# intellerce/controlanimate

Measured on AMD Instinct MI355X. Metric: frames_per_sec, higher is better.
Workload: dtype fp16

## Files before the change

### controlanimate_amd/context.py

```python
from __future__ import annotations

from dataclasses import dataclass, field
from typing import Optional

import torch


@dataclass
class ExecCtx:
    b: int
    f: int
    dtype: torch.dtype
    temb: torch.Tensor
    emb_groups: int
    ehs: Optional[torch.Tensor] = None
    frames_per_kv: int = 1
    kv_mod: int = 0
    gn_frames_per_stat: int = 1
    cache: dict = field(default_factory=dict)

    @property
    def images(self) -> int:
        return self.b * self.f

    def rows_per_emb_group(self, h: int, w: int) -> int:
        return self.images // self.emb_groups * h * w


class Dispatch:
    gemm_ar = True
    ff_fused = True
    tattn_fused = True
    xattn_fused = True
    attn_out_fused = True
    xattn_ip_fused = True
    conv_winograd = True
    gn_winograd = True
    ln_row_sums = True
    repeat_kernel = True
    ln_fold = True
    cfg_shared = True
    cn_cfg_dedup = True
    controlnet_streams = 2


dispatch = Dispatch()
```

### controlanimate_amd/csrc/ca_conv_wino.h

```cpp

template <int DT>
__global__ __launch_bounds__(256) void k_pack_w_wino(const u16* __restrict__ w, u16* __restrict__ dst, int cout, int cin) {
  const int64_t idx = (int64_t)blockIdx.x * 256 + threadIdx.x;
  if (idx >= (int64_t)cout * cin) return;
  const int ci = (int)(idx % cin);
  const int co = (int)(idx / cin);
  float g[3][3];
#pragma unroll
  for (int kh = 0; kh < 3; ++kh)
#pragma unroll
    for (int kw = 0; kw < 3; ++kw) g[kh][kw] = Elem<DT>::to_f(w[((int64_t)co * 9 + kh * 3 + kw) * cin + ci]);
  float t[4][3];
#pragma unroll
  for (int kw = 0; kw < 3; ++kw) {
    t[0][kw] = g[0][kw];
    t[1][kw] = 0.5f * ((g[0][kw] + g[1][kw]) + g[2][kw]);
    t[2][kw] = 0.5f * ((g[0][kw] - g[1][kw]) + g[2][kw]);
    t[3][kw] = g[2][kw];
  }
#pragma unroll
  for (int xi = 0; xi < 4; ++xi) {
    const float u[4] = {t[xi][0], 0.5f * ((t[xi][0] + t[xi][1]) + t[xi][2]), 0.5f * ((t[xi][0] - t[xi][1]) + t[xi][2]), t[xi][2]};
#pragma unroll
    for (int nu = 0; nu < 4; ++nu) dst[((int64_t)(xi * 4 + nu) * cout + co) * cin + ci] = Elem<DT>::from_f(u[nu]);
  }
}

struct WinoParams {
  const u16* x;
  const u16* x2;
  u16* v;
  const u16* mm;
  u16* y;
  const float* bias;
  const float* rowbias;
  const u16* res;
  int64_t ld_res, ld_rowbias;
  int images, h, w, c1, c2, cout;
  int ups;
  int rows_per_group;
  float alpha, post;
  int act;
};

__device__ __forceinline__ unsigned wino_pk_add(unsigned a, unsigned b) {
  unsigned r;
  asm("v_pk_add_f16 %0, %1, %2" : "=v"(r) : "v"(a), "v"(b));
  return r;
}
__device__ __forceinline__ unsigned wino_pk_sub(unsigned a, unsigned b) {
  unsigned r;
  asm("v_pk_add_f16 %0, %1, %2 neg_lo:[0,1] neg_hi:[0,1]" : "=v"(r) : "v"(a), "v"(b));
  return r;
}

template <int DT>
__device__ __forceinline__ unsigned wino_add2(unsigned a, unsigned b) {
  if (DT == CA_F16) return wino_pk_add(a, b);
  return pack2<DT>(Elem<DT>::to_f((u16)(a & 0xffffu)) + Elem<DT>::to_f((u16)(b & 0xffffu)), Elem<DT>::to_f((u16)(a >> 16)) + Elem<DT>::to_f((u16)(b >> 16)));
}
template <int DT>
__device__ __forceinline__ unsigned wino_sub2(unsigned a, unsigned b) {
  if (DT == CA_F16) return wino_pk_sub(a, b);
  return pack2<DT>(Elem<DT>::to_f((u16)(a & 0xffffu)) - Elem<DT>::to_f((u16)(b & 0xffffu)), Elem<DT>::to_f((u16)(a >> 16)) - Elem<DT>::to_f((u16)(b >> 16)));
}

template <int DT>
__global__ __launch_bounds__(256) void k_wino_in(WinoParams p) {
  const int c = p.c1 + p.c2;
  const int chunks = c >> 3;
  const int th = p.h >> 1, tw = p.w >> 1;
  const int64_t tiles = (int64_t)p.images * th * tw;
  const int64_t idx = (int64_t)blockIdx.x * 256 + threadIdx.x;
  if (idx >= tiles * chunks) return;
  const int ck = (int)(idx % chunks);
  const int64_t t = idx / chunks;
  const int tx = (int)(t % tw);
  const int ty = (int)((t / tw) % th);
  const int img = (int)(t / ((int64_t)tw * th));
  const bool second = ck * 8 >= p.c1;
  const u16* src = second ? p.x2 : p.x;
  const int cs = second ? p.c2 : p.c1;
  const int c0 = second ? ck * 8 - p.c1 : ck * 8;
  u32x4 d[4][4];
#pragma unroll
  for (int i = 0; i < 4; ++i) {
    const int hy = 2 * ty - 1 + i;
#pragma unroll
    for (int j = 0; j < 4; ++j) {
      const int wx = 2 * tx - 1 + j;
      const int sh = p.h >> p.ups, sw = p.w >> p.ups;
      d[i][j] = (hy >= 0 && hy < p.h && wx >= 0 && wx < p.w) ? ld16(src + (((int64_t)img * sh + (hy >> p.ups)) * sw + (wx >> p.ups)) * cs + c0) : (u32x4){0u, 0u, 0u, 0u};
    }
  }
  u32x4 r[4][4];
#pragma unroll
  for (int j = 0; j < 4; ++j)
#pragma unroll
    for (int e = 0; e < 4; ++e) {
      r[0][j][e] = wino_sub2<DT>(d[0][j][e], d[2][j][e]);
      r[1][j][e] = wino_add2<DT>(d[1][j][e], d[2][j][e]);
      r[2][j][e] = wino_sub2<DT>(d[2][j][e], d[1][j][e]);
      r[3][j][e] = wino_sub2<DT>(d[1][j][e], d[3][j][e]);
    }
  const int64_t fstride = tiles * c;
  u16* dst = p.v + t * c + ck * 8;
#pragma unroll
  for (int xi = 0; xi < 4; ++xi) {
    u32x4 o[4];
#pragma unroll
    for (int e = 0; e < 4; ++e) {
      o[0][e] = wino_sub2<DT>(r[xi][0][e], r[xi][2][e]);
      o[1][e] = wino_add2<DT>(r[xi][1][e], r[xi][2][e]);
      o[2][e] = wino_sub2<DT>(r[xi][2][e], r[xi][1][e]);
      o[3][e] = wino_sub2<DT>(r[xi][1][e], r[xi][3][e]);
    }
#pragma unroll
    for (int nu = 0; nu < 4; ++nu) st16(dst + (int64_t)(xi * 4 + nu) * fstride, o[nu]);
  }
}

template <int DT>
__global__ __launch_bounds__(256) void k_wino_out(WinoParams p) {
  const int chunks = p.cout >> 3;
  const int th = p.h >> 1, tw = p.w >> 1;
  const int64_t tiles = (int64_t)p.images * th * tw;
  const int64_t idx = (int64_t)blockIdx.x * 256 + threadIdx.x;
  if (idx >= tiles * chunks) return;
  const int ck = (int)(idx % chunks);
  const int64_t t = idx / chunks;
  const int tx = (int)(t % tw);
  const int ty = (int)((t / tw) % th);
  const int img = (int)(t / ((int64_t)tw * th));
  const int64_t fstride = tiles * p.cout;
  const u16* src = p.mm + t * p.cout + ck * 8;
  float s[2][4][8];
#pragma unroll
  for (int nu = 0; nu < 4; ++nu) {
    float m[4][8];
#pragma unroll
    for (int xi = 0; xi < 4; ++xi) unpack8<DT>(ld16(src + (int64_t)(xi * 4 + nu) * fstride), m[xi]);
#pragma unroll
    for (int e = 0; e < 8; ++e) {
      s[0][nu][e] = (m[0][e] + m[1][e]) + m[2][e];
      s[1][nu][e] = (m[1][e] - m[2][e]) - m[3][e];
    }
  }
  const int n0 = ck * 8;
  float bi[8];
#pragma unroll
  for (int e = 0; e < 8; ++e) bi[e] = p.bias ? p.bias[n0 + e] : 0.f;
#pragma unroll
  for (int i = 0; i < 2; ++i)
#pragma unroll
    for (int j = 0; j < 2; ++j) {
      const int64_t m = ((int64_t)img * p.h + 2 * ty + i) * p.w + 2 * tx + j;
      float v[8];
#pragma unroll
      for (int e = 0; e < 8; ++e) v[e] = j == 0 ? (s[i][0][e] + s[i][1][e]) + s[i][2][e] : (s[i][1][e] - s[i][2][e]) - s[i][3][e];
#pragma unroll
      for (int e = 0; e < 8; ++e) v[e] += bi[e];
      if (p.rowbias) {
        const float* rb = p.rowbias + (m / p.rows_per_group) * p.ld_rowbias + n0;
#pragma unroll
        for (int e = 0; e < 8; ++e) v[e] += rb[e];
      }
#pragma unroll
      for (int e = 0; e < 8; ++e) v[e] *= p.alpha;
      if (p.res) {
        float rr[8];
        unpack8<DT>(ld16(p.res + m * p.ld_res + n0), rr);
#pragma unroll
// ... 12 lines not shown
```

### controlanimate_amd/csrc/ca_norm.hip

```cpp
#include "ca_common.h"
#include <stdlib.h>

namespace {

constexpr int GN_MAX_SLOTS = 5;
constexpr int GN_MAX_C = 64 * 8 * GN_MAX_SLOTS;

inline int gn_chunks_rows(int64_t rows_per_stat, int rows_per_chunk) {
  int64_t n = (rows_per_stat + rows_per_chunk - 1) / rows_per_chunk;
  if (n < 16) n = (rows_per_stat + 3) / 4 < 16 ? (rows_per_stat + 3) / 4 : 16;
  if (n < 1) n = 1;
  if (n > 256) n = 256;
  return (int)n;
}
inline int gn_chunks_host(int64_t rows_per_stat) { return gn_chunks_rows(rows_per_stat, 256); }

struct GnParams {
  const u16* x;
  const u16* x2;
  u16* y;
  const float* gamma;
  const float* beta;
  float* partials;
  int c1, c2, groups;
  int64_t rows_per_stat;
  int nchunks;
  int64_t rows_per_chunk;
  float eps;
  int act;
  u16* wino_v;
  int wino_h, wino_w;
};

__host__ __device__ inline int gn_txlog(int c8) {
  int best = 6, best_waste = 1 << 30, best_slots = 0;
  for (int l = 3; l <= 6; ++l) {
    const int tx = 1 << l, slots = (c8 + tx - 1) / tx;
    if (slots > 5) continue;
    const int waste = slots * tx - c8;
    if (waste < best_waste || (waste == best_waste && best_slots != 2 && slots == 2)) {
      best_waste = waste;
      best = l;
      best_slots = slots;
    }
  }
  return best;
}

template <int DT, int txlog, int SLOTS = GN_MAX_SLOTS>
__global__ __launch_bounds__(256) void k_gn_stats(GnParams p) {
  __shared__ float ch_s[GN_MAX_C];
  __shared__ float ch_ss[GN_MAX_C];
  const int C = p.c1 + p.c2, C8 = C >> 3;
// ... 89 lines not shown
      float* out = p.partials + (((int64_t)sg * p.nchunks + chunk) * p.groups + g) * 2;
      out[0] = a;
      out[1] = b;
    }
    return;
  }
#pragma unroll
  for (int k = 0; k < SLOTS; ++k) {
    if ((k << txlog) < C8) {
#pragma unroll
      for (int j = 0; j < 8; ++j) {
#pragma unroll
        for (int off = TX; off < 64; off <<= 1) {
          s[k][j] += __shfl_xor(s[k][j], off);
          ss[k][j] += __shfl_xor(ss[k][j], off);
        }
      }
    }
  }
  for (int w = 0; w < 4; ++w) {
    if (wave == w && lane < TX) {
#pragma unroll
      for (int k = 0; k < SLOTS; ++k) {
        const int c8 = tx + (k << txlog);
        if (c8 < C8) {
#pragma unroll
          for (int j = 0; j < 8; ++j) {
            const int ch = (c8 << 3) + j;
            if (w == 0) {
              ch_s[ch] = s[k][j];
              ch_ss[ch] = ss[k][j];
            } else {
              ch_s[ch] += s[k][j];
              ch_ss[ch] += ss[k][j];
            }
          }
        }
      }
    }
    __syncthreads();
  }
  if (threadIdx.x < p.groups) {
    float a = 0.f, b = 0.f;
    for (int j = 0; j < cpg; ++j) {
      a += ch_s[threadIdx.x * cpg + j];
      b += ch_ss[threadIdx.x * cpg + j];
    }
    float* out = p.partials + (((int64_t)sg * p.nchunks + chunk) * p.groups + threadIdx.x) * 2;
    out[0] = a;
    out[1] = b;
  }
}

template <int DT, int txlog, int SLOTS = GN_MAX_SLOTS>
__global__ __launch_bounds__(256) void k_gn_apply(GnParams p) {
  __shared__ double red[8][64][2];
  __shared__ float gm[64], gr[64];
  const int C = p.c1 + p.c2, C8 = C >> 3;
  constexpr int TX = 1 << txlog, TY = 256 >> txlog;
  const int tx = threadIdx.x & (TX - 1), ty = threadIdx.x >> txlog;
  const int chunk = blockIdx.x, sg = blockIdx.y;
  const int cpg = C / p.groups;
  {
    const int S = p.groups <= 32 ? 8 : 4;
    const int g = threadIdx.x % (256 / S), slot = threadIdx.x / (256 / S);
    if (g < p.groups) {
      double a = 0.0, b = 0.0;
      const float* part = p.partials + ((int64_t)sg * p.nchunks * p.groups + g) * 2;
      for (int k = slot; k < p.nchunks; k += S) {
        const float2 v = *reinterpret_cast<const float2*>(part + (int64_t)k * p.groups * 2);
        a += (double)v.x;
        b += (double)v.y;
      }
      red[slot][g][0] = a;
      red[slot][g][1] = b;
    }
    __syncthreads();
    if (threadIdx.x < p.groups) {
      double a = 0.0, b = 0.0;
      for (int q = 0; q < S; ++q) {
        a += red[q][threadIdx.x][0];
        b += red[q][threadIdx.x][1];
      }
      const double cnt = (double)p.rows_per_stat * (double)cpg;
      const double mean = a / cnt;
      double var = b / cnt - mean * mean;
      if (var < 0.0) var = 0.0;
      gm[threadIdx.x] = (float)mean;
      gr[threadIdx.x] = (float)(1.0 / sqrt(var + (double)p.eps));
    }
    __syncthreads();
  }
  float rs[SLOTS][8], rh[SLOTS][8];
#pragma unroll
  for (int k = 0; k < SLOTS; ++k) {
    const int c8 = tx + (k << txlog);
    if (c8 < C8) {
      const f32x4 g0 = *reinterpret_cast<const f32x4*>(p.gamma + (c8 << 3)), g1 = *reinterpret_cast<const f32x4*>(p.gamma + (c8 << 3) + 4);
      const f32x4 b0 = *reinterpret_cast<const f32x4*>(p.beta + (c8 << 3)), b1 = *reinterpret_cast<const f32x4*>(p.beta + (c8 << 3) + 4);
#pragma unroll
      for (int j = 0; j < 8; ++j) {
        const int gi = ((c8 << 3) + j) / cpg;
        const float scale = gr[gi] * (j < 4 ? g0[j & 3] : g1[j & 3]);
        rs[k][j] = scale;
        rh[k][j] = (j < 4 ? b0[j & 3] : b1[j & 3]) - gm[gi] * scale;
      }
    }
  }
  const int64_t r0 = (int64_t)chunk * p.rows_per_chunk;
  int64_t r1 = r0 + p.rows_per_chunk;
  if (r1 > p.rows_per_stat) r1 = p.rows_per_stat;
  const int64_t base_row = (int64_t)sg * p.rows_per_stat;
  for (int64_t piece = chunk;; piece += 2 * (int64_t)gridDim.x) {
    const int64_t ra = piece * TY + ty, rb = (piece + gridDim.x) * TY + ty;
    if (piece * TY >= p.rows_per_stat) break;
    const bool ok[2] = {ra < p.rows_per_stat, rb < p.rows_per_stat};
    const int64_t rows2[2] = {base_row + ra, base_row + rb};
    u32x4 raw[2][SLOTS];
#pragma unroll
    for (int h = 0; h < 2; ++h)
#pragma unroll
      for (int k = 0; k < SLOTS; ++k) {
        const int c8 = tx + (k << txlog);
        if (c8 < C8 && ok[h]) {
          const int ch = c8 << 3;
          const int64_t rr = rows2[h];
          raw[h][k] = ld16(ch < p.c1 ? p.x + rr * p.c1 + ch : p.x2 + rr * p.c2 + (ch - p.c1));
        }
      }
#pragma unroll
    for (int h = 0; h < 2; ++h)
#pragma unroll
      for (int k = 0; k < SLOTS; ++k) {
        const int c8 = tx + (k << txlog);
        if (c8 < C8 && ok[h]) {
          float f[8];
          unpack8<DT>(raw[h][k], f);
#pragma unroll
          for (int j = 0; j < 8; ++j) {
            const float v = f[j] * rs[k][j] + rh[k][j];
            f[j] = p.act == CA_ACT_SILU ? silu_f(v) : v;
          }
          st16(p.y + rows2[h] * C + (c8 << 3), pack8<DT>(f));
        }
      }
  }
}

constexpr int GNS_MAX = 12;
template <int DT, int NCH = GNS_MAX>
__global__ __launch_bounds__(256) void k_gn_small(GnParams p) {
  __shared__ double red[4][2];
  __shared__ float mr[2];
  const int C = p.c1 + p.c2;
  const int cpg = C / p.groups, q = cpg >> 3;
  const int g = blockIdx.x, sg = blockIdx.y;
  const int total = (int)p.rows_per_stat * q;
  const int64_t base_row = (int64_t)sg * p.rows_per_stat;
  const int lane = threadIdx.x & 63, wave = threadIdx.x >> 6;
  u32x4 raw[NCH];
  float s = 0.f, ss = 0.f;
#pragma unroll
  for (int k = 0; k < NCH; ++k) {
    const int id = threadIdx.x + k * 256;
    if (id < total) {
      const int row = id / q, ch = g * cpg + (id - row * q) * 8;
      const int64_t rr = base_row + row;
      raw[k] = ld16(ch < p.c1 ? p.x + rr * p.c1 + ch : p.x2 + rr * p.c2 + (ch - p.c1));
    }
  }
#pragma unroll
  for (int k = 0; k < NCH; ++k) {
    if (threadIdx.x + k * 256 < total) {
      float f[8];
      unpack8<DT>(raw[k], f);
#pragma unroll
      for (int j = 0; j < 8; ++j) {
        s += f[j];
        ss += f[j] * f[j];
      }
    }
  }
#pragma unroll
  for (int off = 1; off < 64; off <<= 1) {
    s += __shfl_xor(s, off);
    ss += __shfl_xor(ss, off);
  }
  if (lane == 0) {
    red[wave][0] = (double)s;
    red[wave][1] = (double)ss;
  }
  __syncthreads();
  if (threadIdx.x == 0) {
    const double a = red[0][0] + red[1][0] + red[2][0] + red[3][0], b = red[0][1] + red[1][1] + red[2][1] + red[3][1];
    const double cnt = (double)p.rows_per_stat * (double)cpg;
    const double mean = a / cnt;
    double var = b / cnt - mean * mean;
    if (var < 0.0) var = 0.0;
    mr[0] = (float)mean;
    mr[1] = (float)(1.0 / sqrt(var + (double)p.eps));
  }
  __syncthreads();
  const float mean = mr[0], rstd = mr[1];
#pragma unroll
  for (int k = 0; k < NCH; ++k) {
    const int id = threadIdx.x + k * 256;
    if (id < total) {
      const int row = id / q, ch = g * cpg + (id - row * q) * 8;
      const f32x4 g0 = *reinterpret_cast<const f32x4*>(p.gamma + ch), g1 = *reinterpret_cast<const f32x4*>(p.gamma + ch + 4);
      const f32x4 b0 = *reinterpret_cast<const f32x4*>(p.beta + ch), b1 = *reinterpret_cast<const f32x4*>(p.beta + ch + 4);
      float f[8];
      unpack8<DT>(raw[k], f);
#pragma unroll
      for (int j = 0; j < 8; ++j) {
        const float scale = rstd * (j < 4 ? g0[j & 3] : g1[j & 3]);
        const float v = f[j] * scale + ((j < 4 ? b0[j & 3] : b1[j & 3]) - mean * scale);
        f[j] = p.act == CA_ACT_SILU ? silu_f(v) : v;
      }
      st16(p.y + (base_row + row) * C + ch, pack8<DT>(f));
    }
  }
}

__device__ __forceinline__ unsigned gnw_pk_add(unsigned a, unsigned b) {
  unsigned r;
  asm("v_pk_add_f16 %0, %1, %2" : "=v"(r) : "v"(a), "v"(b));
  return r;
}
__device__ __forceinline__ unsigned gnw_pk_sub(unsigned a, unsigned b) {
  unsigned r;
  asm("v_pk_add_f16 %0, %1, %2 neg_lo:[0,1] neg_hi:[0,1]" : "=v"(r) : "v"(a), "v"(b));
  return r;
}
constexpr int GNW_MAX_ROWS = 256, GNW_MAX_CPG = 80;
template <int NCH, int CPG_MAX>
__global__ __launch_bounds__(256) void k_gn_small_wino(GnParams p) {
  constexpr int DT = CA_F16;
  __shared__ double red[4][2];
  __shared__ float mr[2];
  __shared__ __attribute__((aligned(16))) u16 slab[GNW_MAX_ROWS * CPG_MAX];
  const int C = p.c1 + p.c2;
  const int cpg = C / p.groups, q = cpg >> 3;
  const int g = blockIdx.x, sg = blockIdx.y;
  const int total = (int)p.rows_per_stat * q;
  const int64_t base_row = (int64_t)sg * p.rows_per_stat;
  const int lane = threadIdx.x & 63, wave = threadIdx.x >> 6;
  u32x4 raw[NCH];
  float s = 0.f, ss = 0.f;
#pragma unroll
  for (int k = 0; k < NCH; ++k) {
    const int id = threadIdx.x + k * 256;
    if (id < total) {
      const int row = id / q, ch = g * cpg + (id - row * q) * 8;
      const int64_t rr = base_row + row;
      raw[k] = ld16(ch < p.c1 ? p.x + rr * p.c1 + ch : p.x2 + rr * p.c2 + (ch - p.c1));
    }
  }
#pragma unroll
  for (int k = 0; k < NCH; ++k) {
    if (threadIdx.x + k * 256 < total) {
      float f[8];
      unpack8<DT>(raw[k], f);
#pragma unroll
      for (int j = 0; j < 8; ++j) {
        s += f[j];
        ss += f[j] * f[j];
      }
    }
  }
#pragma unroll
  for (int off = 1; off < 64; off <<= 1) {
    s += __shfl_xor(s, off);
    ss += __shfl_xor(ss, off);
  }
  if (lane == 0) {
    red[wave][0] = (double)s;
    red[wave][1] = (double)ss;
  }
  __syncthreads();
  if (threadIdx.x == 0) {
    const double a = red[0][0] + red[1][0] + red[2][0] + red[3][0], b = red[0][1] + red[1][1] + red[2][1] + red[3][1];
    const double cnt = (double)p.rows_per_stat * (double)cpg;
    const double mean = a / cnt;
    double var = b / cnt - mean * mean;
    if (var < 0.0) var = 0.0;
    mr[0] = (float)mean;
    mr[1] = (float)(1.0 / sqrt(var + (double)p.eps));
  }
  __syncthreads();
  const float mean = mr[0], rstd = mr[1];
#pragma unroll
  for (int k = 0; k < NCH; ++k) {
    const int id = threadIdx.x + k * 256;
    if (id < total) {
      const int row = id / q, cq = id - row * q, ch = g * cpg + cq * 8;
      const f32x4 g0 = *reinterpret_cast<const f32x4*>(p.gamma + ch), g1 = *reinterpret_cast<const f32x4*>(p.gamma + ch + 4);
      const f32x4 b0 = *reinterpret_cast<const f32x4*>(p.beta + ch), b1 = *reinterpret_cast<const f32x4*>(p.beta + ch + 4);
      float f[8];
      unpack8<DT>(raw[k], f);
#pragma unroll
      for (int j = 0; j < 8; ++j) {
        const float scale = rstd * (j < 4 ? g0[j & 3] : g1[j & 3]);
        const float v = f[j] * scale + ((j < 4 ? b0[j & 3] : b1[j & 3]) - mean * scale);
        f[j] = p.act == CA_ACT_SILU ? silu_f(v) : v;
      }
      st16(slab + (row * q + cq) * 8, pack8<DT>(f));
    }
  }
  __syncthreads();
  const int th = p.wino_h >> 1, tw = p.wino_w >> 1;
  const int items = th * tw * q;
  const int64_t tiles_total = (int64_t)gridDim.y * th * tw;
  const int64_t fstride = tiles_total * C;
  for (int it = threadIdx.x; it < items; it += 256) {
    const int cq = it % q, t = it / q;
    const int tx = t % tw, ty = t / tw;
    u32x4 d[4][4];
#pragma unroll
    for (int i = 0; i < 4; ++i) {
      const int hy = 2 * ty - 1 + i;
#pragma unroll
      for (int j = 0; j < 4; ++j) {
        const int wx = 2 * tx - 1 + j;
        d[i][j] = (hy >= 0 && hy < p.wino_h && wx >= 0 && wx < p.wino_w) ? ld16(slab + ((hy * p.wino_w + wx) * q + cq) * 8) : (u32x4){0u, 0u, 0u, 0u};
      }
    }
    u32x4 r[4][4];
#pragma unroll
    for (int j = 0; j < 4; ++j)
#pragma unroll
      for (int e = 0; e < 4; ++e) {
        r[0][j][e] = gnw_pk_sub(d[0][j][e], d[2][j][e]);
        r[1][j][e] = gnw_pk_add(d[1][j][e], d[2][j][e]);
        r[2][j][e] = gnw_pk_sub(d[2][j][e], d[1][j][e]);
        r[3][j][e] = gnw_pk_sub(d[1][j][e], d[3][j][e]);
      }
    u16* dst = p.wino_v + ((int64_t)sg * th * tw + t) * C + g * cpg + cq * 8;
#pragma unroll
    for (int xi = 0; xi < 4; ++xi) {
      u32x4 o[4];
#pragma unroll
      for (int e = 0; e < 4; ++e) {
        o[0][e] = gnw_pk_sub(r[xi][0][e], r[xi][2][e]);
        o[1][e] = gnw_pk_add(r[xi][1][e], r[xi][2][e]);
        o[2][e] = gnw_pk_sub(r[xi][2][e], r[xi][1][e]);
        o[3][e] = gnw_pk_sub(r[xi][1][e], r[xi][3][e]);
      }
#pragma unroll
      for (int nu = 0; nu < 4; ++nu) st16(dst + (int64_t)(xi * 4 + nu) * fstride, o[nu]);
    }
  }
}

constexpr int GNU_MAX = 20;
template <int DT, int NCH>
__global__ __launch_bounds__(1024, NCH <= 5 ? 2 : 1) void k_gn_unit(GnParams p, int uc, int units) {
  __shared__ float red[16][4][2];
  __shared__ float mr[4][2];
  __shared__ __attribute__((aligned(16))) float sc[128], sh[128];
  const int C = p.c1 + p.c2;
  const int cpg = C / p.groups, q = uc >> 3, ug = uc / cpg;
  const unsigned bid = blockIdx.x;
  const int nstat = gridDim.x / units;
  int unit, sg;
  if (nstat % 8 == 0) {
    unit = (bid >> 3) % units;
    sg = (bid & 7) + 8 * (bid / (8 * units));
  } else {
    unit = bid % units;
    sg = bid / units;
  }
  const int total = (int)p.rows_per_stat * q;
  const int64_t base_row = (int64_t)sg * p.rows_per_stat;
  const int lane = threadIdx.x & 63, wave = threadIdx.x >> 6;
  u32x4 raw[NCH];
#pragma unroll
  for (int k = 0; k < NCH; ++k) {
    const int id = threadIdx.x + k * 1024;
    if (id < total) {
      const int row = id / q, ch = unit * uc + (id - row * q) * 8;
      const int64_t rr = base_row + row;
      raw[k] = ld16(ch < p.c1 ? p.x + rr * p.c1 + ch : p.x2 + rr * p.c2 + (ch - p.c1));
    }
  }
  float acc[4][2] = {{0.f, 0.f}, {0.f, 0.f}, {0.f, 0.f}, {0.f, 0.f}};
#pragma unroll
  for (int k = 0; k < NCH; ++k) {
    const int id = threadIdx.x + k * 1024;
    if (id < total) {
      const int cq = id % q;
      const int ga = (cq * 8) / cpg, n0 = (ga + 1) * cpg - cq * 8;
      float f[8];
      unpack8<DT>(raw[k], f);
      float lo = 0.f, lo2 = 0.f, hi = 0.f, hi2 = 0.f;
#pragma unroll
      for (int j = 0; j < 8; ++j) {
        if (j < n0) {
          lo += f[j];
          lo2 = fmaf(f[j], f[j], lo2);
        } else {
          hi += f[j];
          hi2 = fmaf(f[j], f[j], hi2);
        }
// ... 310 lines not shown

template <int DT, int L>
void launch_gn_l(bool apply, int slots, const GnParams& p, dim3 grid, hipStream_t st) {
  if (slots <= 2) {
    if (apply) hipLaunchKernelGGL((k_gn_apply<DT, L, 2>), grid, dim3(256), 0, st, p);
    else hipLaunchKernelGGL((k_gn_stats<DT, L, 2>), grid, dim3(256), 0, st, p);
  } else if (slots <= 4) {
    if (apply) hipLaunchKernelGGL((k_gn_apply<DT, L, 4>), grid, dim3(256), 0, st, p);
    else hipLaunchKernelGGL((k_gn_stats<DT, L, 4>), grid, dim3(256), 0, st, p);
  } else {
    if (apply) hipLaunchKernelGGL((k_gn_apply<DT, L, 5>), grid, dim3(256), 0, st, p);
    else hipLaunchKernelGGL((k_gn_stats<DT, L, 5>), grid, dim3(256), 0, st, p);
  }
}

template <int DT>
void launch_gn(bool apply, const GnParams& p, dim3 grid, hipStream_t st) {
  const int c8 = (p.c1 + p.c2) >> 3;
  const int txlog = gn_txlog(c8);
  const int slots = (c8 + (1 << txlog) - 1) >> txlog;
  switch (txlog) {
    case 3: launch_gn_l<DT, 3>(apply, slots, p, grid, st); break;
    case 4: launch_gn_l<DT, 4>(apply, slots, p, grid, st); break;
    case 5: launch_gn_l<DT, 5>(apply, slots, p, grid, st); break;
    default: launch_gn_l<DT, 6>(apply, slots, p, grid, st);
  }
}

extern "C" int ca_groupnorm_stats(const ca_groupnorm_args* a, void* stream) {
  GnParams p{};
  int rc = gn_fill(a, p, "ca_groupnorm_stats");
  if (rc) return rc;
  dim3 grid(p.nchunks, a->images / a->frames_per_stat);
  if (a->dtype == CA_BF16) launch_gn<CA_BF16>(false, p, grid, (hipStream_t)stream);
  else launch_gn<CA_F16>(false, p, grid, (hipStream_t)stream);
  CA_CHECK_LAUNCH("ca_groupnorm_stats");
  return CA_OK;
}

extern "C" int ca_groupnorm_apply(const ca_groupnorm_args* a, void* stream) {
  GnParams p{};
  int rc = gn_fill(a, p, "ca_groupnorm_apply");
  if (rc) return rc;
  CA_REQUIRE(a->y && a->gamma && a->beta, "ca_groupnorm_apply: null operand");
  const int achunks = gn_chunks_rows(p.rows_per_stat, p.rows_per_stat >= 2048 ? 128 : 64);
  p.rows_per_chunk = (p.rows_per_stat + achunks - 1) / achunks;
  dim3 grid(achunks, a->images / a->frames_per_stat);
  if (a->dtype == CA_BF16) launch_gn<CA_BF16>(true, p, grid, (hipStream_t)stream);
  else launch_gn<CA_F16>(true, p, grid, (hipStream_t)stream);
  CA_CHECK_LAUNCH("ca_groupnorm_apply");
  return CA_OK;
}

extern "C" int ca_groupnorm_wino_supported(const ca_groupnorm_args* a) {
  if (!a || !a->x || !a->gamma || !a->beta || !a->wino_v || a->dtype != CA_F16 || a->frames_per_stat != 1) return 0;
  if (a->images <= 0 || a->c1 <= 0 || a->c1 % 8 || a->c2 < 0 || a->c2 % 8 || (a->c2 && !a->x2) || a->groups <= 0) return 0;
  const int C = a->c1 + a->c2;
  if (C % a->groups) return 0;
  const int cpg = C / a->groups;
  if (cpg % 8 || cpg > GNW_MAX_CPG || (a->c2 != 0 && a->c1 % cpg != 0)) return 0;
  if (a->wino_h < 2 || a->wino_w < 2 || (a->wino_h & 1) || (a->wino_w & 1) || a->wino_h * a->wino_w != a->hw || a->hw > GNW_MAX_ROWS) return 0;
  if ((int64_t)a->hw * (cpg >> 3) > 256 * GNS_MAX) return 0;
  if ((((uintptr_t)a->wino_v | (uintptr_t)a->x | (uintptr_t)a->x2) & 15) != 0) return 0;
  return 1;
}

extern "C" int ca_groupnorm(const ca_groupnorm_args* a, void* stream) {
  GnParams p{};
  if (a && a->wino_v) {
    CA_REQUIRE(ca_groupnorm_wino_supported(a), "ca_groupnorm: wino_v with arguments outside the fused form (fp16, per-image statistics, even image of <= 256 pixels, "
                                                "<= 80 channels per group in whole 8-channel chunks): ask ca_groupnorm_wino_supported() first");
    p.x = (const u16*)a->x;
    p.x2 = (const u16*)a->x2;
    p.gamma = a->gamma;
    p.beta = a->beta;
    p.c1 = a->c1, p.c2 = a->c2, p.groups = a->groups;
    p.rows_per_stat = a->hw;
    p.eps = a->eps;
    p.act = a->act;
    p.wino_v = (u16*)a->wino_v;
    p.wino_h = a->wino_h, p.wino_w = a->wino_w;
    {
      const int cpg_w = (a->c1 + a->c2) / a->groups;
      const int64_t per_thread = ((int64_t)a->hw * (cpg_w >> 3) + 255) / 256;
      const dim3 grid_w(a->groups, a->images);
      hipStream_t st_w = (hipStream_t)stream;
#define CA_GNW_CASE(N)                                                                                  \
  if (cpg_w <= 40) hipLaunchKernelGGL((k_gn_small_wino<N, 40>), grid_w, dim3(256), 0, st_w, p);         \
  else hipLaunchKernelGGL((k_gn_small_wino<N, GNW_MAX_CPG>), grid_w, dim3(256), 0, st_w, p);
      if (per_thread <= 2) { CA_GNW_CASE(2) }
      else if (per_thread <= 5) { CA_GNW_CASE(5) }
      else { CA_GNW_CASE(GNS_MAX) }
#undef CA_GNW_CASE
    }
    CA_CHECK_LAUNCH("ca_groupnorm(wino)");
    return CA_OK;
  }
  int rc = gn_fill(a, p, "ca_groupnorm");
  if (rc) return rc;
  CA_REQUIRE(a->y && a->gamma && a->beta, "ca_groupnorm: null operand");
  if (gn_small_ok(p)) {
    const dim3 grid(p.groups, a->images / a->frames_per_stat);
    const int64_t per_thread = (p.rows_per_stat * ((p.c1 + p.c2) / p.groups >> 3) + 255) / 256;
#define CA_GNS_CASE(N)                                                                                                     \
  if (a->dtype == CA_BF16) hipLaunchKernelGGL((k_gn_small<CA_BF16, N>), grid, dim3(256), 0, (hipStream_t)stream, p);       \
  else hipLaunchKernelGGL((k_gn_small<CA_F16, N>), grid, dim3(256), 0, (hipStream_t)stream, p);
    if (per_thread <= 2) { CA_GNS_CASE(2) }
    else if (per_thread <= 5) { CA_GNS_CASE(5) }
    else { CA_GNS_CASE(GNS_MAX) }
#undef CA_GNS_CASE
    CA_CHECK_LAUNCH("ca_groupnorm");
    return CA_OK;
  }
  if (const int uc = gn_unit_channels(p)) {
    const int units = (p.c1 + p.c2) / uc;
    const dim3 grid(units * (a->images / a->frames_per_stat));
    static const int gnu_small = CA_KNOB("CA_GN_UNIT_SMALL", 1);
    const bool few = gnu_small && (int64_t)p.rows_per_stat * (uc >> 3) <= 1024 * 5;
    if (a->dtype == CA_BF16) {
      if (few) hipLaunchKernelGGL((k_gn_unit<CA_BF16, 5>), grid, dim3(1024), 0, (hipStream_t)stream, p, uc, units);
      else hipLaunchKernelGGL((k_gn_unit<CA_BF16, GNU_MAX>), grid, dim3(1024), 0, (hipStream_t)stream, p, uc, units);
    } else {
      if (few) hipLaunchKernelGGL((k_gn_unit<CA_F16, 5>), grid, dim3(1024), 0, (hipStream_t)stream, p, uc, units);
      else hipLaunchKernelGGL((k_gn_unit<CA_F16, GNU_MAX>), grid, dim3(1024), 0, (hipStream_t)stream, p, uc, units);
// ... 58 lines not shown
```

### controlanimate_amd/kernels.py

```python
from __future__ import annotations

import ctypes as C
from typing import Optional

import torch

from . import _capi
from .context import dispatch
from ._capi import (AttnArgs, ConvArgs, ConvNarrowArgs, FfArgs, TattnArgs, XattnArgs, GemmArgs, GroupNormArgs, LayerNormArgs, CA_ACT_NONE,
                    CA_ACT_SILU, CA_BF16, CA_F16, check, lib)

ACT_NONE, ACT_SILU = CA_ACT_NONE, CA_ACT_SILU
ACT_QUICK_GELU, ACT_GELU = 2, 3


def dt_code(dtype: torch.dtype) -> int:
    if dtype == torch.bfloat16:
        return CA_BF16
    if dtype == torch.float16:
        return CA_F16
    raise TypeError(f"activations must be bf16 or fp16, got {dtype}")


def _stream() -> int:
# ... 231 lines not shown
            rows_per_group: int = 0, residual: Optional[torch.Tensor] = None, stride: int = 1,
            upsample: bool = False, alpha: float = 1.0, post_scale: float = 1.0, act: int = ACT_NONE,
            out_f32: bool = False, pad_asym: bool = False, w_wino: Optional[torch.Tensor] = None) -> torch.Tensor:
    _req_cuda(x, w, x2, bias, rowbias, residual, w_wino)
    assert x.dim() == 4 and x.is_contiguous() and w.dim() == 4 and w.is_contiguous()
    images, hin, win, cin1 = x.shape
    cin2 = 0
    if x2 is not None:
        assert x2.is_contiguous() and x2.shape[:3] == x.shape[:3] and x2.dtype == x.dtype
        cin2 = x2.shape[3]
    cout = w.shape[0]
    assert tuple(w.shape[1:]) == (3, 3, cin1 + cin2) and w.dtype == x.dtype
    hl, wl = (hin * 2, win * 2) if upsample else (hin, win)
    pad = 1 if pad_asym else 2
    hout, wout = (hl + pad - 3) // stride + 1, (wl + pad - 3) // stride + 1
    y = torch.empty((images, hout, wout, cout), device=x.device, dtype=torch.float32 if out_f32 else x.dtype)
    ld_res = 0
    if residual is not None:
        assert residual.dtype == x.dtype and residual.is_contiguous() and residual.numel() == images * hout * wout * cout, \
            f"residual {tuple(residual.shape)} {residual.dtype} contiguous={residual.is_contiguous()} vs output {(images, hout, wout, cout)} {x.dtype}"
        ld_res = cout
    if rowbias is not None:
        assert rowbias.dtype == torch.float32 and rowbias.dim() == 2 and rowbias.shape[1] == cout and rows_per_group > 0
    if bias is not None:
        assert bias.dtype == torch.float32 and bias.numel() == cout
    args = ConvArgs(x=_p(x), x2=_p(x2), w=_p(w), y=_p(y), bias=_p(bias), rowbias=_p(rowbias),
                    residual=_p(residual), ld_res=ld_res,
                    ld_rowbias=rowbias.stride(0) if rowbias is not None else 0, images=images, hin=hin,
                    win=win, cin1=cin1, cin2=cin2, cout=cout, stride=stride, upsample=int(upsample),
                    rows_per_group=rows_per_group, alpha=alpha, post_scale=post_scale, act=act,
                    out_f32=int(out_f32), dtype=dt_code(x.dtype), pad_asym=int(pad_asym))
    if w_wino is not None and dispatch.conv_winograd:
        assert w_wino.dtype == x.dtype and w_wino.is_contiguous() and tuple(w_wino.shape) == (16, cout, cin1 + cin2)
        args.w_wino = _p(w_wino)
    wbytes = int(lib().ca_conv3x3_workspace_bytes(C.byref(args)))
    if wbytes > 0:
        ws = torch.empty((wbytes,), device=x.device, dtype=torch.uint8)
        args.workspace, args.workspace_bytes = _p(ws), wbytes
    _record_plan(lib().ca_conv3x3_plan_name, args)
    check(lib().ca_conv3x3(C.byref(args), _stream()), "ca_conv3x3")
    return y


_gn_wino_declined: dict = {}


def group_norm_conv3x3_wino(x: torch.Tensor, gamma: torch.Tensor, beta: torch.Tensor, w: torch.Tensor, w_wino: torch.Tensor, *,
                            x2: Optional[torch.Tensor] = None, groups: int = 32, eps: float = 1e-5, act: int = ACT_NONE,
                            bias: Optional[torch.Tensor] = None, rowbias: Optional[torch.Tensor] = None, rows_per_group: int = 0,
                            residual: Optional[torch.Tensor] = None, post_scale: float = 1.0) -> Optional[torch.Tensor]:
    if not (dispatch.conv_winograd and dispatch.gn_winograd):
        return None
    _req_cuda(x, gamma, beta, w, w_wino, x2, bias, rowbias, residual)
    if x.dim() != 4 or not x.is_contiguous() or x.dtype != torch.float16 or (x2 is not None and (not x2.is_contiguous() or x2.shape[:3] != x.shape[:3])):
        return None
    images, h, w_, c1 = x.shape
    c2 = 0 if x2 is None else x2.shape[3]
    c, cout = c1 + c2, w.shape[0]
    tiles = images * (h // 2) * (w_ // 2)
    key = (images, h, w_, c1, c2, cout, groups, act, rowbias is not None, residual is not None, rows_per_group)
    if _gn_wino_declined.get(key):
        return None
    cargs = ConvArgs(x=_p(x), x2=None, w=_p(w), y=_p(x), bias=_p(bias), rowbias=_p(rowbias), residual=_p(residual),
                     ld_res=cout if residual is not None else 0, ld_rowbias=rowbias.stride(0) if rowbias is not None else 0, images=images, hin=h,
                     win=w_, cin1=c, cin2=0, cout=cout, stride=1, upsample=0, rows_per_group=rows_per_group, alpha=1.0, post_scale=post_scale,
                     act=ACT_NONE, out_f32=0, dtype=dt_code(x.dtype), pad_asym=0, w_wino=_p(w_wino), x_is_wino_v=1)
    cargs.workspace, cargs.workspace_bytes = _p(x), 1 << 60
    buf = C.create_string_buffer(64)
    if lib().ca_conv3x3_plan_name(C.byref(cargs), buf, 64) != 0 or not buf.value.decode().startswith("wino"):
        _gn_wino_declined[key] = True
        return None
    wbytes = int(lib().ca_conv3x3_workspace_bytes(C.byref(cargs)))
    gargs = GroupNormArgs(x=_p(x), x2=_p(x2), y=None, gamma=_p(gamma), beta=_p(beta), partials=None, images=images, hw=h * w_, c1=c1, c2=c2,
                          groups=groups, frames_per_stat=1, eps=eps, act=act, dtype=dt_code(x.dtype), wino_v=_p(x), wino_h=h, wino_w=w_)
    if wbytes <= 0 or not lib().ca_groupnorm_wino_supported(C.byref(gargs)):
        _gn_wino_declined[key] = True
        return None
    y = torch.empty((images, h, w_, cout), device=x.device, dtype=x.dtype)
    v = torch.empty((16, tiles, c), device=x.device, dtype=x.dtype)
    if residual is not None:
        assert residual.dtype == x.dtype and residual.is_contiguous() and residual.numel() == y.numel()
    ws = torch.empty((wbytes,), device=x.device, dtype=torch.uint8)
    cargs.x, cargs.y, gargs.wino_v = _p(v), _p(y), _p(v)
    cargs.workspace, cargs.workspace_bytes = _p(ws), wbytes
    if _plan_sink is not None:
        buf = C.create_string_buffer(64)
        _plan_sink.append("gn_" + (buf.value.decode() if lib().ca_conv3x3_plan_name(C.byref(cargs), buf, 64) == 0 else "?"))
    check(lib().ca_groupnorm(C.byref(gargs), _stream()), "ca_groupnorm(wino)")
    check(lib().ca_conv3x3(C.byref(cargs), _stream()), "ca_conv3x3(wino, V given)")
    return y


def group_norm(x: torch.Tensor, gamma: torch.Tensor, beta: torch.Tensor, *, x2: Optional[torch.Tensor] = None,
               groups: int = 32, frames_per_stat: int = 1, eps: float = 1e-5, act: int = ACT_NONE) -> torch.Tensor:
    _req_cuda(x, gamma, beta, x2)
    assert x.dim() == 4 and x.is_contiguous()
    images, h, w_, c1 = x.shape
    c2 = 0
    if x2 is not None:
        assert x2.is_contiguous() and x2.shape[:3] == x.shape[:3] and x2.dtype == x.dtype
        c2 = x2.shape[3]
    c = c1 + c2
    assert gamma.dtype == torch.float32 and beta.dtype == torch.float32 and gamma.numel() == c and beta.numel() == c
    y = torch.empty((images, h, w_, c), device=x.device, dtype=x.dtype)
    nfl = lib().ca_groupnorm_partials_floats(images, h * w_, frames_per_stat, groups)
    partials = torch.empty((max(int(nfl), 1),), device=x.device, dtype=torch.float32)
    args = GroupNormArgs(x=_p(x), x2=_p(x2), y=_p(y), gamma=_p(gamma), beta=_p(beta), partials=_p(partials),
                         images=images, hw=h * w_, c1=c1, c2=c2, groups=groups,
                         frames_per_stat=frames_per_stat, eps=eps, act=act, dtype=dt_code(x.dtype))
    check(lib().ca_groupnorm(C.byref(args), _stream()), "ca_groupnorm")
    return y


def layer_norm(x: torch.Tensor, gamma: torch.Tensor, beta: torch.Tensor, *, pos: Optional[torch.Tensor] = None,
               rows_per_frame: int = 1, frames: int = 1, eps: float = 1e-5) -> torch.Tensor:
    _req_cuda(x, gamma, beta, pos)
    assert x.dim() == 2 and x.is_contiguous()
    rows, c = x.shape
    assert gamma.dtype == torch.float32 and beta.dtype == torch.float32
    if pos is not None:
        assert pos.dtype == torch.float32 and pos.is_contiguous() and pos.shape == (frames, c)
    y = torch.empty_like(x)
    args = LayerNormArgs(x=_p(x), y=_p(y), gamma=_p(gamma), beta=_p(beta), pos=_p(pos), rows=rows, c=c,
                         rows_per_frame=rows_per_frame, frames=frames, eps=eps, dtype=dt_code(x.dtype))
    check(lib().ca_layernorm(C.byref(args), _stream()), "ca_layernorm")
    return y


def row_stats(x: torch.Tensor, eps: float = 1e-5) -> torch.Tensor:
    _req_cuda(x)
    assert x.dim() == 2 and x.is_contiguous()
    rows, c = x.shape
    st = torch.empty((rows, 2), device=x.device, dtype=torch.float32)
    args = LayerNormArgs(x=_p(x), y=None, gamma=None, beta=None, pos=None, rows=rows, c=c, rows_per_frame=1, frames=1,
                         eps=eps, dtype=dt_code(x.dtype), stats=_p(st))
    check(lib().ca_layernorm(C.byref(args), _stream()), "ca_layernorm(stats)")
    return st


def attention_raw(q: torch.Tensor, k: torch.Tensor, v: torch.Tensor, o: torch.Tensor, *, q_off: int, k_off: int,
# ... 364 lines not shown
```

Baseline: 15.71.

## Add two-pass GroupNorm that writes Winograd V directly for larger images

Adds a kernel that takes precomputed GroupNorm statistics, normalizes a band of rows into shared memory, and applies the Winograd input transform straight into V. This extends the fused GN+Winograd path beyond the small-image single-launch form, and to bf16. The goal is to skip writing the normalized activation and reading it back in a separate winograd-input pass. The common transform is factored into a shared helper. In exchange, halo rows are loaded again for each band, shared-memory usage is large, and the stats pass stays a separate launch.

```diff
diff --git a/controlanimate_amd/context.py b/controlanimate_amd/context.py
--- a/controlanimate_amd/context.py
+++ b/controlanimate_amd/context.py
@@ -36,6 +36,7 @@
     xattn_ip_fused = True
     conv_winograd = True
     gn_winograd = True
+    gn_winograd_twopass = True
     ln_row_sums = True
     repeat_kernel = True
     ln_fold = True
diff --git a/controlanimate_amd/csrc/ca_conv_wino.h b/controlanimate_amd/csrc/ca_conv_wino.h
--- a/controlanimate_amd/csrc/ca_conv_wino.h
+++ b/controlanimate_amd/csrc/ca_conv_wino.h
@@ -66,6 +66,33 @@
 }
 
 template <int DT>
+__device__ __forceinline__ void wino_bt_d_b(const u32x4 (&d)[4][4], u16* dst, int64_t fstride) {
+  u32x4 r[4][4];
+#pragma unroll
+  for (int j = 0; j < 4; ++j)
+#pragma unroll
+    for (int e = 0; e < 4; ++e) {
+      r[0][j][e] = wino_sub2<DT>(d[0][j][e], d[2][j][e]);
+      r[1][j][e] = wino_add2<DT>(d[1][j][e], d[2][j][e]);
+      r[2][j][e] = wino_sub2<DT>(d[2][j][e], d[1][j][e]);
+      r[3][j][e] = wino_sub2<DT>(d[1][j][e], d[3][j][e]);
+    }
+#pragma unroll
+  for (int xi = 0; xi < 4; ++xi) {
+    u32x4 o[4];
+#pragma unroll
+    for (int e = 0; e < 4; ++e) {
+      o[0][e] = wino_sub2<DT>(r[xi][0][e], r[xi][2][e]);
+      o[1][e] = wino_add2<DT>(r[xi][1][e], r[xi][2][e]);
+      o[2][e] = wino_sub2<DT>(r[xi][2][e], r[xi][1][e]);
+      o[3][e] = wino_sub2<DT>(r[xi][1][e], r[xi][3][e]);
+    }
+#pragma unroll
+    for (int nu = 0; nu < 4; ++nu) st16(dst + (int64_t)(xi * 4 + nu) * fstride, o[nu]);
+  }
+}
+
+template <int DT>
 __global__ __launch_bounds__(256) void k_wino_in(WinoParams p) {
   const int c = p.c1 + p.c2;
   const int chunks = c >> 3;
@@ -93,31 +120,7 @@
       d[i][j] = (hy >= 0 && hy < p.h && wx >= 0 && wx < p.w) ? ld16(src + (((int64_t)img * sh + (hy >> p.ups)) * sw + (wx >> p.ups)) * cs + c0) : (u32x4){0u, 0u, 0u, 0u};
     }
   }
-  u32x4 r[4][4];
-#pragma unroll
-  for (int j = 0; j < 4; ++j)
-#pragma unroll
-    for (int e = 0; e < 4; ++e) {
-      r[0][j][e] = wino_sub2<DT>(d[0][j][e], d[2][j][e]);
-      r[1][j][e] = wino_add2<DT>(d[1][j][e], d[2][j][e]);
-      r[2][j][e] = wino_sub2<DT>(d[2][j][e], d[1][j][e]);
-      r[3][j][e] = wino_sub2<DT>(d[1][j][e], d[3][j][e]);
-    }
-  const int64_t fstride = tiles * c;
-  u16* dst = p.v + t * c + ck * 8;
-#pragma unroll
-  for (int xi = 0; xi < 4; ++xi) {
-    u32x4 o[4];
-#pragma unroll
-    for (int e = 0; e < 4; ++e) {
-      o[0][e] = wino_sub2<DT>(r[xi][0][e], r[xi][2][e]);
-      o[1][e] = wino_add2<DT>(r[xi][1][e], r[xi][2][e]);
-      o[2][e] = wino_sub2<DT>(r[xi][2][e], r[xi][1][e]);
-      o[3][e] = wino_sub2<DT>(r[xi][1][e], r[xi][3][e]);
-    }
-#pragma unroll
-    for (int nu = 0; nu < 4; ++nu) st16(dst + (int64_t)(xi * 4 + nu) * fstride, o[nu]);
-  }
+  wino_bt_d_b<DT>(d, p.v + t * c + ck * 8, tiles * c);
 }
 
 template <int DT>
diff --git a/controlanimate_amd/csrc/ca_norm.hip b/controlanimate_amd/csrc/ca_norm.hip
--- a/controlanimate_amd/csrc/ca_norm.hip
+++ b/controlanimate_amd/csrc/ca_norm.hip
@@ -1,4 +1,5 @@
 #include "ca_common.h"
+#include "ca_conv_wino.h"
 #include <stdlib.h>
 
 namespace {
@@ -194,6 +195,63 @@
   }
 }
 
+__device__ __forceinline__ void gn_group_stats(const GnParams& p, int sg, int cpg, double (*red)[64][2], float* gm, float* gr) {
+  const int S = p.groups <= 32 ? 8 : 4;
+  const int g = threadIdx.x % (256 / S), slot = threadIdx.x / (256 / S);
+  if (g < p.groups) {
+    double a = 0.0, b = 0.0;
+    const float* part = p.partials + ((int64_t)sg * p.nchunks * p.groups + g) * 2;
+    for (int k = slot; k < p.nchunks; k += S) {
+      const float2 v = *reinterpret_cast<const float2*>(part + (int64_t)k * p.groups * 2);
+      a += (double)v.x;
+      b += (double)v.y;
+    }
+    red[slot][g][0] = a;
+    red[slot][g][1] = b;
+  }
+  __syncthreads();
+  if (threadIdx.x < p.groups) {
+    double a = 0.0, b = 0.0;
+    for (int q = 0; q < S; ++q) {
+      a += red[q][threadIdx.x][0];
+      b += red[q][threadIdx.x][1];
+    }
+    const double cnt = (double)p.rows_per_stat * (double)cpg;
+    const double mean = a / cnt;
+    double var = b / cnt - mean * mean;
+    if (var < 0.0) var = 0.0;
+    gm[threadIdx.x] = (float)mean;
+    gr[threadIdx.x] = (float)(1.0 / sqrt(var + (double)p.eps));
+  }
+  __syncthreads();
+}
+
+template <bool FMA = false>
+__device__ __forceinline__ void gn_scale_shift(const GnParams& p, int c8, int cpg, const float* gm, const float* gr, float* rs, float* rh) {
+  const f32x4 g0 = *reinterpret_cast<const f32x4*>(p.gamma + (c8 << 3)), g1 = *reinterpret_cast<const f32x4*>(p.gamma + (c8 << 3) + 4);
+  const f32x4 b0 = *reinterpret_cast<const f32x4*>(p.beta + (c8 << 3)), b1 = *reinterpret_cast<const f32x4*>(p.beta + (c8 << 3) + 4);
+#pragma unroll
+  for (int j = 0; j < 8; ++j) {
+    const int gi = ((c8 << 3) + j) / cpg;
+    const float scale = gr[gi] * (j < 4 ? g0[j & 3] : g1[j & 3]);
+    rs[j] = scale;
+    const float b = j < 4 ? b0[j & 3] : b1[j & 3];
+    rh[j] = FMA ? fmaf(-gm[gi], scale, b) : b - gm[gi] * scale;
+  }
+}
+
+template <int DT, bool FMA = false>
+__device__ __forceinline__ u32x4 gn_norm8(u32x4 raw, const float* rs, const float* rh, int act) {
+  float f[8];
+  unpack8<DT>(raw, f);
+#pragma unroll
+  for (int j = 0; j < 8; ++j) {
+    const float v = FMA ? fmaf(f[j], rs[j], rh[j]) : f[j] * rs[j] + rh[j];
+    f[j] = act == CA_ACT_SILU ? silu_f(v) : v;
+  }
+  return pack8<DT>(f);
+}
+
 template <int DT, int txlog, int SLOTS = GN_MAX_SLOTS>
 __global__ __launch_bounds__(256) void k_gn_apply(GnParams p) {
   __shared__ double red[8][64][2];
@@ -203,51 +261,12 @@
   const int tx = threadIdx.x & (TX - 1), ty = threadIdx.x >> txlog;
   const int chunk = blockIdx.x, sg = blockIdx.y;
   const int cpg = C / p.groups;
-  {
-    const int S = p.groups <= 32 ? 8 : 4;
-    const int g = threadIdx.x % (256 / S), slot = threadIdx.x / (256 / S);
-    if (g < p.groups) {
-      double a = 0.0, b = 0.0;
-      const float* part = p.partials + ((int64_t)sg * p.nchunks * p.groups + g) * 2;
-      for (int k = slot; k < p.nchunks; k += S) {
-        const float2 v = *reinterpret_cast<const float2*>(part + (int64_t)k * p.groups * 2);
-        a += (double)v.x;
-        b += (double)v.y;
-      }
-      red[slot][g][0] = a;
-      red[slot][g][1] = b;
-    }
-    __syncthreads();
-    if (threadIdx.x < p.groups) {
-      double a = 0.0, b = 0.0;
-      for (int q = 0; q < S; ++q) {
-        a += red[q][threadIdx.x][0];
-        b += red[q][threadIdx.x][1];
-      }
-      const double cnt = (double)p.rows_per_stat * (double)cpg;
-      const double mean = a / cnt;
-      double var = b / cnt - mean * mean;
-      if (var < 0.0) var = 0.0;
-      gm[threadIdx.x] = (float)mean;
-      gr[threadIdx.x] = (float)(1.0 / sqrt(var + (double)p.eps));
-    }
-    __syncthreads();
-  }
+  gn_group_stats(p, sg, cpg, red, gm, gr);
   float rs[SLOTS][8], rh[SLOTS][8];
 #pragma unroll
   for (int k = 0; k < SLOTS; ++k) {
     const int c8 = tx + (k << txlog);
-    if (c8 < C8) {
-      const f32x4 g0 = *reinterpret_cast<const f32x4*>(p.gamma + (c8 << 3)), g1 = *reinterpret_cast<const f32x4*>(p.gamma + (c8 << 3) + 4);
-      const f32x4 b0 = *reinterpret_cast<const f32x4*>(p.beta + (c8 << 3)), b1 = *reinterpret_cast<const f32x4*>(p.beta + (c8 << 3) + 4);
-#pragma unroll
-      for (int j = 0; j < 8; ++j) {
-        const int gi = ((c8 << 3) + j) / cpg;
-        const float scale = gr[gi] * (j < 4 ? g0[j & 3] : g1[j & 3]);
-        rs[k][j] = scale;
-        rh[k][j] = (j < 4 ? b0[j & 3] : b1[j & 3]) - gm[gi] * scale;
-      }
-    }
+    if (c8 < C8) gn_scale_shift(p, c8, cpg, gm, gr, rs[k], rh[k]);
   }
   const int64_t r0 = (int64_t)chunk * p.rows_per_chunk;
   int64_t r1 = r0 + p.rows_per_chunk;
@@ -275,17 +294,73 @@
 #pragma unroll
       for (int k = 0; k < SLOTS; ++k) {
         const int c8 = tx + (k << txlog);
-        if (c8 < C8 && ok[h]) {
-          float f[8];
-          unpack8<DT>(raw[h][k], f);
-#pragma unroll
-          for (int j = 0; j < 8; ++j) {
-            const float v = f[j] * rs[k][j] + rh[k][j];
-            f[j] = p.act == CA_ACT_SILU ? silu_f(v) : v;
-          }
-          st16(p.y + rows2[h] * C + (c8 << 3), pack8<DT>(f));
-        }
-      }
+        if (c8 < C8 && ok[h]) st16(p.y + rows2[h] * C + (c8 << 3), gn_norm8<DT>(raw[h][k], rs[k], rh[k], p.act));
+      }
+  }
+}
+
+constexpr int GAW_CC8 = 8;
+constexpr int GAW_PIX = 320;
+constexpr int GAW_STRIDE = GAW_CC8 * 8 + 8;
+static_assert(GAW_PIX * GAW_STRIDE * 2 >= 8 * 64 * 2 * 8, "the slab also serves as the fp64 scratch of gn_group_stats");
+inline int gaw_band(int h, int w) {
+  const int rows = GAW_PIX / w;
+  if (rows < 4) return 0;
+  const int band = (rows - 2) / 2;
+  return band < (h >> 1) ? band : (h >> 1);
+}
+template <int DT>
+__global__ __launch_bounds__(256) void k_gn_apply_wino(GnParams p, int band) {
+  __shared__ __attribute__((aligned(16))) u16 slab[GAW_PIX * GAW_STRIDE];
+  __shared__ float gm[64], gr[64];
+  const int C = p.c1 + p.c2, C8 = C >> 3, cpg = C / p.groups;
+  const int cblocks = (C8 + GAW_CC8 - 1) / GAW_CC8;
+  const int cb = blockIdx.x % cblocks, bandi = blockIdx.x / cblocks, sg = blockIdx.y;
+  gn_group_stats(p, sg, cpg, reinterpret_cast<double (*)[64][2]>(slab), gm, gr);
+  const int cq = threadIdx.x & (GAW_CC8 - 1), c8 = cb * GAW_CC8 + cq, ch = c8 << 3;
+  const bool cok = c8 < C8;
+  float rs[8], rh[8];
+  if (cok) gn_scale_shift<true>(p, c8, cpg, gm, gr, rs, rh);
+  const int H = p.wino_h, W = p.wino_w, th = H >> 1, tw = W >> 1;
+  const int ty0 = bandi * band, ty1 = ty0 + band < th ? ty0 + band : th;
+  const int row_lo = 2 * ty0 - 1;
+  const int ra = row_lo < 0 ? 0 : row_lo, rb = 2 * ty1 + 1 < H ? 2 * ty1 + 1 : H;
+  const int npix = (rb - ra) * W;
+  const int64_t first = (int64_t)sg * p.rows_per_stat + (int64_t)ra * W;
+  const u16* src = ch < p.c1 ? p.x + first * p.c1 + ch : p.x2 + first * p.c2 + (ch - p.c1);
+  const int ld = ch < p.c1 ? p.c1 : p.c2;
+  u16* srow = slab + (ra - row_lo) * W * GAW_STRIDE + cq * 8;
+  constexpr int PP = 256 / GAW_CC8;
+  for (int px0 = threadIdx.x / GAW_CC8; px0 < npix; px0 += 4 * PP) {
+    u32x4 raw[4];
+#pragma unroll
+    for (int u = 0; u < 4; ++u) {
+      const int px = px0 + u * PP;
+      if (cok && px < npix) raw[u] = ld16(src + (int64_t)px * ld);
+    }
+#pragma unroll
+    for (int u = 0; u < 4; ++u) {
+      const int px = px0 + u * PP;
+      if (cok && px < npix) st16(srow + px * GAW_STRIDE, gn_norm8<DT, true>(raw[u], rs, rh, p.act));
+    }
+  }
+  __syncthreads();
+  const int64_t fstride = (int64_t)gridDim.y * th * tw * C;
+  const int ntl = (ty1 - ty0) * tw;
+  for (int tl = threadIdx.x / GAW_CC8; tl < ntl; tl += PP) {
+    if (!cok) break;
+    const int tx = tl % tw, ty = ty0 + tl / tw;
+    u32x4 d[4][4];
+#pragma unroll
+    for (int i = 0; i < 4; ++i) {
+      const int hy = 2 * ty - 1 + i;
+#pragma unroll
+      for (int j = 0; j < 4; ++j) {
+        const int wx = 2 * tx - 1 + j;
+        d[i][j] = (hy >= 0 && hy < H && wx >= 0 && wx < W) ? ld16(slab + ((hy - row_lo) * W + wx) * GAW_STRIDE + cq * 8) : (u32x4){0u, 0u, 0u, 0u};
+      }
+    }
+    wino_bt_d_b<DT>(d, p.wino_v + (((int64_t)sg * th + ty) * tw + tx) * C + ch, fstride);
   }
 }
 
@@ -364,16 +439,6 @@
   }
 }
 
-__device__ __forceinline__ unsigned gnw_pk_add(unsigned a, unsigned b) {
-  unsigned r;
-  asm("v_pk_add_f16 %0, %1, %2" : "=v"(r) : "v"(a), "v"(b));
-  return r;
-}
-__device__ __forceinline__ unsigned gnw_pk_sub(unsigned a, unsigned b) {
-  unsigned r;
-  asm("v_pk_add_f16 %0, %1, %2 neg_lo:[0,1] neg_hi:[0,1]" : "=v"(r) : "v"(a), "v"(b));
-  return r;
-}
 constexpr int GNW_MAX_ROWS = 256, GNW_MAX_CPG = 80;
 template <int NCH, int CPG_MAX>
 __global__ __launch_bounds__(256) void k_gn_small_wino(GnParams p) {
@@ -467,30 +532,7 @@
         d[i][j] = (hy >= 0 && hy < p.wino_h && wx >= 0 && wx < p.wino_w) ? ld16(slab + ((hy * p.wino_w + wx) * q + cq) * 8) : (u32x4){0u, 0u, 0u, 0u};
       }
     }
-    u32x4 r[4][4];
-#pragma unroll
-    for (int j = 0; j < 4; ++j)
-#pragma unroll
-      for (int e = 0; e < 4; ++e) {
-        r[0][j][e] = gnw_pk_sub(d[0][j][e], d[2][j][e]);
-        r[1][j][e] = gnw_pk_add(d[1][j][e], d[2][j][e]);
-        r[2][j][e] = gnw_pk_sub(d[2][j][e], d[1][j][e]);
-        r[3][j][e] = gnw_pk_sub(d[1][j][e], d[3][j][e]);
-      }
-    u16* dst = p.wino_v + ((int64_t)sg * th * tw + t) * C + g * cpg + cq * 8;
-#pragma unroll
-    for (int xi = 0; xi < 4; ++xi) {
-      u32x4 o[4];
-#pragma unroll
-      for (int e = 0; e < 4; ++e) {
-        o[0][e] = gnw_pk_sub(r[xi][0][e], r[xi][2][e]);
-        o[1][e] = gnw_pk_add(r[xi][1][e], r[xi][2][e]);
-        o[2][e] = gnw_pk_sub(r[xi][2][e], r[xi][1][e]);
-        o[3][e] = gnw_pk_sub(r[xi][1][e], r[xi][3][e]);
-      }
-#pragma unroll
-      for (int nu = 0; nu < 4; ++nu) st16(dst + (int64_t)(xi * 4 + nu) * fstride, o[nu]);
-    }
+    wino_bt_d_b<CA_F16>(d, p.wino_v + ((int64_t)sg * th * tw + t) * C + g * cpg + cq * 8, fstride);
   }
 }
 
@@ -907,7 +949,7 @@
   return CA_OK;
 }
 
-extern "C" int ca_groupnorm_wino_supported(const ca_groupnorm_args* a) {
+static int gn_wino_one_launch_ok(const ca_groupnorm_args* a) {
   if (!a || !a->x || !a->gamma || !a->beta || !a->wino_v || a->dtype != CA_F16 || a->frames_per_stat != 1) return 0;
   if (a->images <= 0 || a->c1 <= 0 || a->c1 % 8 || a->c2 < 0 || a->c2 % 8 || (a->c2 && !a->x2) || a->groups <= 0) return 0;
   const int C = a->c1 + a->c2;
@@ -920,11 +962,48 @@
   return 1;
 }
 
+static int gn_wino_two_pass_ok(const ca_groupnorm_args* a) {
+  if (!a || !a->x || !a->gamma || !a->beta || !a->wino_v || (a->dtype != CA_F16 && a->dtype != CA_BF16) || a->frames_per_stat != 1) return 0;
+  if (a->images <= 0 || a->images > 65535 || a->c1 <= 0 || a->c1 % 8 || a->c2 < 0 || a->c2 % 8 || (a->c2 && !a->x2)) return 0;
+  const int C = a->c1 + a->c2;
+  if (C > GN_MAX_C || a->groups <= 0 || a->groups > 64 || C % a->groups) return 0;
+  if (a->wino_h < 2 || a->wino_w < 2 || (a->wino_h & 1) || (a->wino_w & 1) || (int64_t)a->wino_h * a->wino_w != a->hw) return 0;
+  if (gaw_band(a->wino_h, a->wino_w) < 1) return 0;
+  if ((((uintptr_t)a->wino_v | (uintptr_t)a->x | (uintptr_t)a->x2) & 15) != 0) return 0;
+  GnParams q{};
+  q.y = (u16*)a->wino_v;
+  q.c1 = a->c1, q.c2 = a->c2, q.groups = a->groups;
+  q.rows_per_stat = a->hw;
+  return !gn_small_ok(q) && !gn_unit_channels(q);
+}
+
+extern "C" int ca_groupnorm_wino_supported(const ca_groupnorm_args* a) {
+  if (gn_wino_one_launch_ok(a)) return 1;
+  return gn_wino_two_pass_ok(a) ? 2 : 0;
+}
+
 extern "C" int ca_groupnorm(const ca_groupnorm_args* a, void* stream) {
   GnParams p{};
   if (a && a->wino_v) {
-    CA_REQUIRE(ca_groupnorm_wino_supported(a), "ca_groupnorm: wino_v with arguments outside the fused form (fp16, per-image statistics, even image of <= 256 pixels, "
-                                                "<= 80 channels per group in whole 8-channel chunks): ask ca_groupnorm_wino_supported() first");
+    if (!gn_wino_one_launch_ok(a)) {
+      CA_REQUIRE(gn_wino_two_pass_ok(a), "ca_groupnorm: wino_v with arguments outside both V-writing forms (per-image statistics, an even image; one launch: fp16, "
+                                          "<= 256 pixels, <= 80 channels per group in whole 8-channel chunks; two passes: <= %d pixels per row and a shape the "
+                                          "y-writing call runs in two passes too): ask ca_groupnorm_wino_supported() first", GAW_PIX / 4);
+      int rc = gn_fill(a, p, "ca_groupnorm(wino, two-pass)");
+      if (rc) return rc;
+      rc = ca_groupnorm_stats(a, stream);
+      if (rc) return rc;
+      p.y = nullptr;
+      p.wino_v = (u16*)a->wino_v;
+      p.wino_h = a->wino_h, p.wino_w = a->wino_w;
+      const int band = gaw_band(a->wino_h, a->wino_w);
+      const int cblocks = (((a->c1 + a->c2) >> 3) + GAW_CC8 - 1) / GAW_CC8, bands = ((a->wino_h >> 1) + band - 1) / band;
+      const dim3 grid_t((unsigned)(cblocks * bands), (unsigned)a->images);
+      if (a->dtype == CA_BF16) hipLaunchKernelGGL((k_gn_apply_wino<CA_BF16>), grid_t, dim3(256), 0, (hipStream_t)stream, p, band);
+      else hipLaunchKernelGGL((k_gn_apply_wino<CA_F16>), grid_t, dim3(256), 0, (hipStream_t)stream, p, band);
+      CA_CHECK_LAUNCH("ca_groupnorm(wino, two-pass)");
+      return CA_OK;
+    }
     p.x = (const u16*)a->x;
     p.x2 = (const u16*)a->x2;
     p.gamma = a->gamma;
diff --git a/controlanimate_amd/kernels.py b/controlanimate_amd/kernels.py
--- a/controlanimate_amd/kernels.py
+++ b/controlanimate_amd/kernels.py
@@ -307,13 +307,14 @@
     if not (dispatch.conv_winograd and dispatch.gn_winograd):
         return None
     _req_cuda(x, gamma, beta, w, w_wino, x2, bias, rowbias, residual)
-    if x.dim() != 4 or not x.is_contiguous() or x.dtype != torch.float16 or (x2 is not None and (not x2.is_contiguous() or x2.shape[:3] != x.shape[:3])):
+    if (x.dim() != 4 or not x.is_contiguous() or x.dtype not in (torch.float16, torch.bfloat16)
+            or (x2 is not None and (not x2.is_contiguous() or x2.shape[:3] != x.shape[:3] or x2.dtype != x.dtype))):
         return None
     images, h, w_, c1 = x.shape
     c2 = 0 if x2 is None else x2.shape[3]
     c, cout = c1 + c2, w.shape[0]
     tiles = images * (h // 2) * (w_ // 2)
-    key = (images, h, w_, c1, c2, cout, groups, act, rowbias is not None, residual is not None, rows_per_group)
+    key = (images, h, w_, c1, c2, cout, groups, act, rowbias is not None, residual is not None, rows_per_group, x.dtype, dispatch.gn_winograd_twopass)
     if _gn_wino_declined.get(key):
         return None
     cargs = ConvArgs(x=_p(x), x2=None, w=_p(w), y=_p(x), bias=_p(bias), rowbias=_p(rowbias), residual=_p(residual),
@@ -328,7 +329,8 @@
     wbytes = int(lib().ca_conv3x3_workspace_bytes(C.byref(cargs)))
     gargs = GroupNormArgs(x=_p(x), x2=_p(x2), y=None, gamma=_p(gamma), beta=_p(beta), partials=None, images=images, hw=h * w_, c1=c1, c2=c2,
                           groups=groups, frames_per_stat=1, eps=eps, act=act, dtype=dt_code(x.dtype), wino_v=_p(x), wino_h=h, wino_w=w_)
-    if wbytes <= 0 or not lib().ca_groupnorm_wino_supported(C.byref(gargs)):
+    form = int(lib().ca_groupnorm_wino_supported(C.byref(gargs))) if wbytes > 0 else 0
+    if form == 0 or (form == 2 and not dispatch.gn_winograd_twopass):
         _gn_wino_declined[key] = True
         return None
     y = torch.empty((images, h, w_, cout), device=x.device, dtype=x.dtype)
@@ -338,9 +340,12 @@
     ws = torch.empty((wbytes,), device=x.device, dtype=torch.uint8)
     cargs.x, cargs.y, gargs.wino_v = _p(v), _p(y), _p(v)
     cargs.workspace, cargs.workspace_bytes = _p(ws), wbytes
+    if form == 2:
+        partials = torch.empty((max(int(lib().ca_groupnorm_partials_floats(images, h * w_, 1, groups)), 1),), device=x.device, dtype=torch.float32)
+        gargs.partials = _p(partials)
     if _plan_sink is not None:
         buf = C.create_string_buffer(64)
-        _plan_sink.append("gn_" + (buf.value.decode() if lib().ca_conv3x3_plan_name(C.byref(cargs), buf, 64) == 0 else "?"))
+        _plan_sink.append(("gn_" if form == 1 else "gn2_") + (buf.value.decode() if lib().ca_conv3x3_plan_name(C.byref(cargs), buf, 64) == 0 else "?"))
     check(lib().ca_groupnorm(C.byref(gargs), _stream()), "ca_groupnorm(wino)")
     check(lib().ca_conv3x3(C.byref(cargs), _stream()), "ca_conv3x3(wino, V given)")
     return y
```

After: 15.76, median of 5. About the same (+0.3%).
